# mpc001/auto_avsr

Measured on AMD Instinct MI355X. Metric: video-frames/sec/node (25fps 88x88, max-frames=1600), E2E training step (fwd+bwd+clip+AdamW), higher is better.
Workload: dtype f16 activations x f16x2 weights (atrunk3, atrunk4, decoder, encoder, trunk3, trunk4) + split-bf16 (everything else) forward / bf16 backward

## Files before the change

auto_avsr_amd/csrc/gemm_split.hip:

```cpp
#include "gemm_core.h"
#include "avsr_hip.h"

namespace {

using avsr_gemm_impl::Params;

template <int BM, int BN, int STAGES, int CV, bool BSP = false, int WGM = 2, int WGN = 2, int ACV = 0>
struct SplitKernel {
    static constexpr int BK = 32, NW = WGM * WGN, NTHR = 64 * NW;
    static_assert(NW == 4 || NW == 8, "four or eight waves");
    static constexpr int WM = BM / WGM, WN = BN / WGN, TM = WM / 32, TN = WN / 32;
    static_assert(WM % 32 == 0 && WN % 32 == 0, "wave tile must be a multiple of 32 x 32");
    static constexpr int A_BYTES = BM * 128, B_BYTES = BN * 128, STAGE_BYTES = A_BYTES + B_BYTES;
    static constexpr int A_LOADS = BM / (8 * NW), B_LOADS = BN / (8 * NW);
    static_assert(A_LOADS >= 1 && B_LOADS >= 1 && BM % (8 * NW) == 0 && BN % (8 * NW) == 0, "tile / wave-count mismatch");
    static constexpr int LPT = A_LOADS + B_LOADS;
    static constexpr size_t RING_BYTES = (size_t)STAGES * STAGE_BYTES, EPI_BYTES = (size_t)BM * (BN + 4) * 4;
    static constexpr size_t LDS_BYTES = RING_BYTES > EPI_BYTES ? RING_BYTES : EPI_BYTES;
    static_assert(BM % 64 == 0 && BN % 64 == 0, "tile must be a multiple of 64 x 64");

    struct Rows {
        const float* a[A_LOADS];
        uint32_t mask[A_LOADS];
        const float* b[B_LOADS];
    };

    static AVSR_DEV Rows decode_rows(const Params& p, const float* A, const float* B, int m0, int n0, int wave, int lane) {
        Rows ri;
        const int rsub = lane >> 3, pc = lane & 7;
#pragma unroll
        for (int i = 0; i < A_LOADS; i++) {
            const int r = (wave * A_LOADS + i) * 8 + rsub;
            const int c = pc ^ ((r >> 1) & 7);
            if (CV == 0) {
                const int gr = min(m0 + r, p.M - 1);
                ri.a[i] = A + (size_t)gr * p.lda + c * 4;
                ri.mask[i] = 0;
            } else {
                const int m = min(m0 + r, p.M - 1);
                const int pix = p.cOH * p.cOW;
                const int n = m / pix, rem = m - n * pix;
                const int oh = rem / p.cOW, ow = rem - oh * p.cOW;
                const int ya = oh * p.cS - p.cPH, xa = ow * p.cS - p.cPW;
                ri.a[i] = A + ((long)n * p.cH * p.cW + (long)ya * p.cW + xa) * p.cC + c * 4;
                uint32_t mk = 0;
                for (int t = 0; t < p.cKH * p.cKW; t++) {
                    const int ta = t / p.cKW, tb = t - ta * p.cKW;
                    const int y = ya + ta, x = xa + tb;
                    if (y >= 0 && y < p.cH && x >= 0 && x < p.cW) mk |= 1u << t;
                }
                ri.mask[i] = mk;
            }
        }
#pragma unroll
        for (int i = 0; i < B_LOADS; i++) {
            const int r = (wave * B_LOADS + i) * 8 + rsub;
            const int c = pc ^ ((r >> 1) & 7);
            const int gr = min(n0 + r, p.N - 1);
            ri.b[i] = B + (size_t)gr * p.ldb + c * 4;
        }
        return ri;
    }

    static AVSR_DEV void issue(const Params& p, const Rows& ri, int kbeg, int t, char* stage, int wave) {
        long da, db;
        int tap = 0;
        if (CV == 0) {
            da = db = kbeg + t * BK;
        } else {
            const int cpt = p.cC / BK;
            tap = t / cpt;
            const int cb = (t - tap * cpt) * BK;
            const int ta = tap / p.cKW, tb = tap - ta * p.cKW;
            da = (long)(ta * p.cW + tb) * p.cC + cb;
            db = (long)tap * p.cC + cb;
        }
#pragma unroll
        for (int i = 0; i < A_LOADS; i++) {
            const float* src = ri.a[i] + da;
            if (CV != 0) src = ((ri.mask[i] >> tap) & 1u) ? src : reinterpret_cast<const float*>(p.gate);
            glds16(src, stage + (wave * A_LOADS + i) * 1024);
        }
#pragma unroll
        for (int i = 0; i < B_LOADS; i++) glds16(ri.b[i] + db, stage + A_BYTES + (wave * B_LOADS + i) * 1024);
    }

    static AVSR_DEV Frag<2> frag(const char* base, int r, int half8) {
        const int sw = (r >> 1) & 7;
        const f32x4 a = *reinterpret_cast<const f32x4*>(base + r * 128 + (((2 * half8) ^ sw) << 4));
        const f32x4 b = *reinterpret_cast<const f32x4*>(base + r * 128 + (((2 * half8 + 1) ^ sw) << 4));
        Frag<2> f;
#pragma unroll
        for (int e = 0; e < 4; e++) {
            bf16_t s0[2], s1[2];
            split_bf16<2>(a[e], s0);
            split_bf16<2>(b[e], s1);
            f.p[0][e] = (short)s0[0];
            f.p[1][e] = (short)s0[1];
            f.p[0][e + 4] = (short)s1[0];
            f.p[1][e + 4] = (short)s1[1];
        }
        return f;
    }

    static AVSR_DEV Frag<2> frag_presplit(const char* base, int r, int half8) {
        const int sw = (r >> 1) & 7;
        Frag<2> f;
        f.p[0] = *reinterpret_cast<const bf16x8*>(base + r * 128 + (((2 * half8) ^ sw) << 4));
        f.p[1] = *reinterpret_cast<const bf16x8*>(base + r * 128 + (((2 * half8 + 1) ^ sw) << 4));
        return f;
    }
    static AVSR_DEV void convert_a(char* As) {
#pragma unroll
        for (int j = 0; j < BM * 4 / NTHR; j++) {
            const int idx = threadIdx.x + NTHR * j;
            const int r = idx >> 2, g = idx & 3;
            const Frag<2> f = frag(As, r, g);
            const int sw = (r >> 1) & 7;
            *reinterpret_cast<bf16x8*>(As + r * 128 + (((2 * g) ^ sw) << 4)) = f.p[0];
            *reinterpret_cast<bf16x8*>(As + r * 128 + (((2 * g + 1) ^ sw) << 4)) = f.p[1];
        }
    }

    static AVSR_DEV void run(const Params& p, char* smem) {
        const float* A = reinterpret_cast<const float*>(p.A);
        const float* B = reinterpret_cast<const float*>(p.B);
        const int lane = threadIdx.x & 63, wave = wave_id();
        const int wm = wave / WGN, wn = wave % WGN;
        const int m0 = blockIdx.y * BM, n0 = blockIdx.x * BN;
        const int zs = blockIdx.z;
        int kbeg = 0, nt;
        if (CV == 0) {
            kbeg = zs * p.k_chunk;
            nt = (min(p.K, kbeg + p.k_chunk) - kbeg) / BK;
        } else {
            nt = p.cKH * p.cKW * (p.cC / BK);
        }
        f32x16 acc[TM][TN];
#pragma unroll
        for (int i = 0; i < TM; i++)
#pragma unroll
            for (int j = 0; j < TN; j++)
#pragma unroll
                for (int r = 0; r < 16; r++) acc[i][j][r] = 0.f;

        const Rows ri = decode_rows(p, A, B, m0, n0, wave, lane);
#pragma unroll
        for (int s = 0; s < STAGES - 1; s++)
            if (s < nt) issue(p, ri, kbeg, s, smem + s * STAGE_BYTES, wave);

        auto step = [&](int t, auto issue_flag) {
            constexpr bool ISSUE = decltype(issue_flag)::value;
            if (ISSUE) {
                wait_vmcnt<(STAGES - 2) * LPT>();
            } else {
                switch (nt - 1 - t) {
                    case 0: wait_vmcnt<0>(); break;
                    default: wait_vmcnt<(STAGES > 2 ? LPT : 0)>(); break;
                }
            }
            block_barrier_raw();
            char* As = smem + (t % STAGES) * STAGE_BYTES;
            const char* Bs = As + A_BYTES;
            if (ACV == 1) {
                convert_a(As);
                lds_wait<0>();
                sched_fence();
                block_barrier_raw();
            }
            const int arow = wm * WM + (lane & 31), brow = wn * WN + (lane & 31);
            Frag<2> fa[TM], fb[TN];
            auto load_frags = [&](int ks) {
                const int h8 = ks * 2 + (lane >> 5);
#pragma unroll
                for (int i = 0; i < TM; i++) fa[i] = ACV ? frag_presplit(As, arow + i * 32, h8) : frag(As, arow + i * 32, h8);
#pragma unroll
                for (int j = 0; j < TN; j++) fb[j] = BSP ? frag_presplit(Bs, brow + j * 32, h8) : frag(Bs, brow + j * 32, h8);
            };
            load_frags(0);
            sched_fence();
            if (ISSUE) issue(p, ri, kbeg, t + STAGES - 1, smem + ((t + STAGES - 1) % STAGES) * STAGE_BYTES, wave);
            sched_fence();
#pragma unroll
            for (int ks = 0; ks < BK / 16; ks++) {
#pragma unroll
                for (int i = 0; i < TM; i++)
#pragma unroll
                    for (int j = 0; j < TN; j++) acc[i][j] = mfma32(fa[i].p[1], fb[j].p[0], acc[i][j]);
#pragma unroll
                for (int i = 0; i < TM; i++)
#pragma unroll
                    for (int j = 0; j < TN; j++) acc[i][j] = mfma32(fa[i].p[0], fb[j].p[1], acc[i][j]);
#pragma unroll
                for (int i = 0; i < TM; i++)
#pragma unroll
                    for (int j = 0; j < TN; j++) acc[i][j] = mfma32(fa[i].p[0], fb[j].p[0], acc[i][j]);
                if (ks + 1 < BK / 16) load_frags(ks + 1);
            }
        };
        int t = 0;
        for (; t + STAGES - 1 < nt; t++) step(t, std::true_type{});
        for (; t < nt; t++) step(t, std::false_type{});
        if (CV != 0) {
            Params q = p;
            q.gate = nullptr;
            avsr_gemm_impl::epilogue_lds<BM, BN, TM, TN, NTHR, 1>(acc, q, m0, n0, wm * WM, wn * WN, zs, 0, smem);
            if (BM > 128 && p.colstat && blockIdx.x == 0) {
                const int r2 = (int)gridDim.y + (int)blockIdx.y;
                if (r2 < p.colstat_rows)
                    for (int i = threadIdx.x; i < 2 * p.N; i += NTHR) p.colstat[(size_t)r2 * 2 * p.N + i] = 0.f;
            }
        } else {
            avsr_gemm_impl::epilogue_lds<BM, BN, TM, TN, NTHR, 1>(acc, p, m0, n0, wm * WM, wn * WN, zs, 0, smem);
        }
    }
};

template <int BM, int BN, int STAGES, int CV, bool BSP, int WGM, int WGN, int ACV>
__global__ __launch_bounds__(64 * WGM * WGN) void gemm_split_kernel(Params p) {
    AVSR_DYN_SMEM(smem);
    SplitKernel<BM, BN, STAGES, CV, BSP, WGM, WGN, ACV>::run(p, smem);
}

template <int BM, int BN, int STAGES, int CV, bool BSP, int WGM = 2, int WGN = 2, int ACV = 0>
void launch_split(Params& p, int split_k, hipStream_t stream) {
    using K = SplitKernel<BM, BN, STAGES, CV, BSP, WGM, WGN, ACV>;
    if (CV == 0) {
        int kc = (p.K + split_k - 1) / split_k;
        kc = ((kc + 31) / 32) * 32;
        split_k = (p.K + kc - 1) / kc;
        p.k_chunk = kc;
    } else {
        split_k = 1;
    }
    dim3 grid((p.N + BN - 1) / BN, (p.M + BM - 1) / BM, split_k), block(K::NTHR);
    AVSR_LAUNCH((gemm_split_kernel<BM, BN, STAGES, CV, BSP, WGM, WGN, ACV>), grid, block, K::LDS_BYTES, stream, p);
}

template <int CV, bool BSP>
bool launch_tile(int tile, Params& p, int split_k, hipStream_t stream) {
    switch (tile) {
        case 11: launch_split<64, 64, 3, CV, BSP, 2, 2, 1>(p, split_k, stream); return true;
        case 12: launch_split<64, 64, 2, CV, BSP, 2, 2, 1>(p, split_k, stream); return true;
        case 13: launch_split<128, 64, 2, CV, BSP, 2, 2, 1>(p, split_k, stream); return true;
        case 14: launch_split<128, 128, 2, CV, BSP, 2, 2, 1>(p, split_k, stream); return true;
        case 15: launch_split<128, 64, 3, CV, BSP, 2, 2, 1>(p, split_k, stream); return true;
        case 16: launch_split<128, 128, 3, CV, BSP, 2, 2, 1>(p, split_k, stream); return true;
        case 23: if constexpr (BSP) { launch_split<128, 64, 2, CV, BSP, 2, 2, 2>(p, split_k, stream); return true; } return false;
        case 24: if constexpr (BSP) { launch_split<128, 128, 2, CV, BSP, 2, 2, 2>(p, split_k, stream); return true; } return false;
        case 25: if constexpr (BSP) { launch_split<128, 64, 3, CV, BSP, 2, 2, 2>(p, split_k, stream); return true; } return false;
        case 26: if constexpr (BSP) { launch_split<128, 128, 3, CV, BSP, 2, 2, 2>(p, split_k, stream); return true; } return false;
        case 27: if constexpr (BSP) { launch_split<256, 64, 2, CV, BSP, 4, 2, 2>(p, split_k, stream); return true; } return false;
        case 28: if constexpr (BSP) { launch_split<256, 64, 3, CV, BSP, 4, 2, 2>(p, split_k, stream); return true; } return false;
        case 29: if constexpr (BSP) { launch_split<256, 128, 3, CV, BSP, 4, 2, 2>(p, split_k, stream); return true; } return false;
        case 30: if constexpr (BSP) { launch_split<256, 128, 2, CV, BSP, 4, 2, 2>(p, split_k, stream); return true; } return false;
        case 1: launch_split<64, 64, 3, CV, BSP>(p, split_k, stream); return true;
        case 2: launch_split<64, 64, 2, CV, BSP>(p, split_k, stream); return true;
        case 3: launch_split<128, 64, 2, CV, BSP>(p, split_k, stream); return true;
        case 4: launch_split<128, 128, 2, CV, BSP>(p, split_k, stream); return true;
        case 5: launch_split<128, 64, 3, CV, BSP>(p, split_k, stream); return true;
        case 6: launch_split<128, 128, 3, CV, BSP>(p, split_k, stream); return true;
        case 7: launch_split<128, 64, 2, CV, BSP, 4, 1>(p, split_k, stream); return true;
        default: return false;
    }
}

__global__ __launch_bounds__(256) void split_pack_kernel(const float* __restrict__ src, bf16_t* __restrict__ dst, long n8) {
    for (long i = (long)blockIdx.x * 256 + threadIdx.x; i < n8; i += (long)gridDim.x * 256) {
        float v[8];
        load8(src + i * 8, v);
        bf16x8 hi, lo;
#pragma unroll
        for (int e = 0; e < 8; e++) {
            bf16_t pl[2];
            split_bf16<2>(v[e], pl);
            hi[e] = (short)pl[0];
            lo[e] = (short)pl[1];
        }
        *reinterpret_cast<bf16x8*>(dst + i * 16) = hi;
        *reinterpret_cast<bf16x8*>(dst + i * 16 + 8) = lo;
    }
}
struct AvsrSplitEntry {
    const float* src;
    bf16_t* dst;
    long n8;
    long blk0;
};
__global__ __launch_bounds__(256) void multi_split_pack_kernel(const AvsrSplitEntry* __restrict__ table, int n) {
    int lo_ = 0, hi_ = n - 1;
    while (lo_ < hi_) {
        const int mid = (lo_ + hi_ + 1) >> 1;
        if (table[mid].blk0 <= (long)blockIdx.x) lo_ = mid; else hi_ = mid - 1;
    }
    const AvsrSplitEntry e = table[lo_];
    const long i = ((long)blockIdx.x - e.blk0) * 256 + threadIdx.x;
    if (i >= e.n8) return;
    float v[8];
    load8(e.src + i * 8, v);
    bf16x8 hi, lo;
#pragma unroll
    for (int k = 0; k < 8; k++) {
        bf16_t pl[2];
        split_bf16<2>(v[k], pl);
        hi[k] = (short)pl[0];
        lo[k] = (short)pl[1];
    }
    *reinterpret_cast<bf16x8*>(e.dst + i * 16) = hi;
    *reinterpret_cast<bf16x8*>(e.dst + i * 16 + 8) = lo;
}

}

extern "C" int avsr_gemm_f32s_nt(const float* A, int lda, const float* B, int ldb, int M, int N, int K, const float* bias,
                                 int act, const void* gate, int gate_dtype, int ldg, float gate_scale, float drop_p,
                                 uint64_t seed, const uint64_t* seed_dev, float alpha, const float* alpha_dev,
                                 const void* resid, int resid_dtype, int ldr, void* C, int c_dtype, int ldc, int accumulate,
                                 int split_k, int tile, float* colsum, int b_split, void* c2, int ldc2, hipStream_t stream) {
    AVSR_REQUIRE(!(colsum && accumulate), "gemm_f32s_nt: colsum needs a non-accumulating output");
    AVSR_REQUIRE(!(c2 && (accumulate || c_dtype != 0)), "gemm_f32s_nt: the bf16 twin needs a non-accumulating f32 output");
    AVSR_REQUIRE(K > 0 && K % 64 == 0, "gemm_f32s_nt: K must be a positive multiple of 64");
    AVSR_REQUIRE(lda % 4 == 0 && ldb % 4 == 0, "gemm_f32s_nt: lda/ldb must be multiples of 4 elements");
    AVSR_REQUIRE(((uintptr_t)A % 16) == 0 && ((uintptr_t)B % 16) == 0, "gemm_f32s_nt: operands must be 16-byte aligned");
    AVSR_REQUIRE(!(accumulate && c_dtype != 0), "gemm_f32s_nt: accumulate needs an f32 output");
    AVSR_REQUIRE(!(split_k > 1 && !accumulate), "gemm_f32s_nt: split-K needs accumulate=1");
    if (M <= 0 || N <= 0) return 0;
    Params p{};
    p.A = A; p.B = B; p.lda = lda; p.ldb = ldb;
    p.M = M; p.N = N; p.K = K;
    p.bias = bias; p.act = act;
    p.gate = gate; p.gate_dtype = gate_dtype; p.ldg = ldg; p.gate_scale = gate_scale;
    p.drop_p = drop_p; p.seed = seed; p.seed_dev = seed_dev;
    p.alpha = alpha; p.alpha_dev = alpha_dev;
    p.resid = reinterpret_cast<const float*>(resid); p.resid_dtype = resid_dtype; p.ldr = ldr;
    p.C = C; p.c_dtype = c_dtype; p.ldc = ldc; p.accumulate = accumulate;
    p.colsum = colsum;
    p.C2 = c2; p.ldc2 = ldc2;
    p.nsplit = 1; p.batch_h = 1; p.nbatch = 1;
    if (split_k < 1) split_k = 1;
    float* colsum_det = nullptr;
    if (avsr_det()) {
        split_k = 1;
        if (colsum) {
            AVSR_REQUIRE(ldc == N, "gemm_f32s_nt (deterministic mode): colsum needs a dense output");
            colsum_det = colsum;
            p.colsum = nullptr;
        }
    }
    if (tile == 0) {
        const long t128 = (long)((M + 127) / 128) * ((N + 127) / 128);
        const long t12864 = (long)((M + 127) / 128) * ((N + 63) / 64);
        tile = t128 >= 1024 ? 14 : (t12864 >= 400 ? 13 : 11);
    }
    const bool ok = b_split ? launch_tile<0, true>(tile, p, split_k, stream) : launch_tile<0, false>(tile, p, split_k, stream);
    AVSR_REQUIRE(ok, "gemm_f32s_nt: unknown tile code");
    if (colsum_det) avsr_colsum_det(C, c_dtype, ldc, M, N, colsum_det, stream);
    AVSR_CHECK_LAUNCH("gemm_f32s_nt");
    return 0;
}

static int conv2d_f32s_impl(const float* x, const float* wp, float* y, const void* zero_page, int N, int H, int W, int Cin, int Cout, int KH,
                            int KW, int stride, int pad_h, int pad_w, int tile, int w_split, void* y2, float* stats_part, int stats_tiles,
                            hipStream_t stream) {
    const int OH = (H + 2 * pad_h - KH) / stride + 1, OW = (W + 2 * pad_w - KW) / stride + 1;
    AVSR_REQUIRE(Cin % 64 == 0, "conv2d_f32s: input channel count must be a multiple of 64");
    AVSR_REQUIRE(zero_page != nullptr, "conv2d_f32s: zero page required");
    AVSR_REQUIRE(KH * KW <= 32, "conv2d_f32s: at most 32 filter taps");
    AVSR_REQUIRE((long)N * H * W < (1l << 31) && (long)N * OH * OW < (1l << 31), "conv2d_f32s: pixel count exceeds int32");
    AVSR_REQUIRE(stats_part == nullptr || (long)stats_tiles * 128 >= (long)N * OH * OW, "conv2d_f32s: statistics buffer too small");
    if (N <= 0) return 0;
    Params p{};
    p.A = x; p.B = wp;
    p.K = KH * KW * Cin; p.lda = Cin; p.ldb = p.K;
    p.alpha = 1.f; p.gate_scale = 1.f;
    p.nsplit = 1; p.batch_h = 1; p.nbatch = 1;
    p.gate = zero_page;
    p.c_dtype = 0; p.C = y;
    p.C2 = y2; p.ldc2 = Cout;
    p.cN = N;
    p.cKH = KH; p.cKW = KW; p.cS = stride; p.cPH = pad_h; p.cPW = pad_w; p.cC = Cin;
    p.M = N * OH * OW; p.N = Cout; p.ldc = Cout;
    p.cH = H; p.cW = W; p.cOH = OH; p.cOW = OW;
    p.colstat = stats_part;
    p.colstat_rows = stats_tiles;
    if (tile == 0) tile = Cout >= 128 ? 14 : 13;
    if (tile == 23 && avsr_tune_knobs[21] == 0 && Cout == 64 && (long)N * OH * OW >= 65536) tile = 27;
    if (tile == 23 && avsr_tune_knobs[21] > 0) tile = avsr_tune_knobs[21];
    if (tile == 24 && avsr_tune_knobs[22] > 0) tile = avsr_tune_knobs[22];
    AVSR_REQUIRE(stats_part == nullptr || tile == 13 || tile == 14 || (tile >= 23 && tile <= 30), "conv2d_f32s: statistics need a 128- or 256-row tile");
    const bool ok = w_split ? launch_tile<1, true>(tile, p, 1, stream) : launch_tile<1, false>(tile, p, 1, stream);
    AVSR_REQUIRE(ok, "conv2d_f32s: unknown tile code");
    AVSR_CHECK_LAUNCH("conv2d_f32s");
    return 0;
}

extern "C" int avsr_conv2d_f32s(const float* x, const float* wp, float* y, const void* zero_page, int N, int H, int W, int Cin,
                                int Cout, int KH, int KW, int stride, int pad_h, int pad_w, int tile, int w_split, void* y2,
                                hipStream_t stream) {
    return conv2d_f32s_impl(x, wp, y, zero_page, N, H, W, Cin, Cout, KH, KW, stride, pad_h, pad_w, tile, w_split, y2, nullptr, 0, stream);
}

extern "C" int avsr_conv2d_f32s_stats(const float* x, const float* wp, float* y, const void* zero_page, int N, int H, int W, int Cin,
                                      int Cout, int KH, int KW, int stride, int pad_h, int pad_w, int tile, int w_split, void* y2,
                                      float* stats_part, int stats_tiles, hipStream_t stream) {
    AVSR_REQUIRE(stats_part != nullptr, "conv2d_f32s_stats: statistics buffer required");
    return conv2d_f32s_impl(x, wp, y, zero_page, N, H, W, Cin, Cout, KH, KW, stride, pad_h, pad_w, tile, w_split, y2, stats_part, stats_tiles, stream);
}

extern "C" int avsr_split_pack(const float* src, void* dst, int64_t n, hipStream_t stream) {
    AVSR_REQUIRE(n % 8 == 0, "split_pack: element count must be a multiple of 8");
    AVSR_REQUIRE(((uintptr_t)src % 16) == 0 && ((uintptr_t)dst % 16) == 0, "split_pack: 16-byte aligned buffers");
    if (n <= 0) return 0;
    const long n8 = n / 8, nb = (n8 + 255) / 256;
    AVSR_LAUNCH(split_pack_kernel, dim3((unsigned)(nb > 4096 ? 4096 : nb)), dim3(256), 0, stream, src, (bf16_t*)dst, n8);
    AVSR_CHECK_LAUNCH("split_pack");
    return 0;
}

extern "C" int avsr_multi_split_pack(const void* table, int n, int total_blocks, hipStream_t stream) {
    if (n <= 0 || total_blocks <= 0) return 0;
    AVSR_LAUNCH(multi_split_pack_kernel, dim3(total_blocks), dim3(256), 0, stream, reinterpret_cast<const AvsrSplitEntry*>(table), n);
    AVSR_CHECK_LAUNCH("multi_split_pack");
    return 0;
}
```

Baseline: 69900.

## Add persistent direct 3x3 C64 split-bf16 conv kernel with halo patch staging

Adds a dedicated persistent kernel for 3x3 stride-1 64-to-64 channel convolutions with split-bf16 weights. It keeps the high weight half in registers and the low half in LDS, and stages haloed input row-bands into a double-buffered, swizzled LDS patch. The patch loads are woven into the MFMA loop, and the epilogue fuses the bf16 copy and BN statistics. It replaces the generic implicit-GEMM tile path, cutting redundant im2col loads and weight reloads. The cost is a complex hand-scheduled kernel with heavy register use and large LDS.

```diff
diff --git a/auto_avsr_amd/csrc/conv3x3_c64_split.hip b/auto_avsr_amd/csrc/conv3x3_c64_split.hip
--- /dev/null
+++ b/auto_avsr_amd/csrc/conv3x3_c64_split.hip
@@ -0,0 +1,330 @@
+#include "prims.h"
+#include "avsr_hip.h"
+
+namespace {
+
+template <class T> AVSR_DEV void opaque(T& v) {
+#ifndef AVSR_EMU
+    asm volatile("" : "+v"(v));
+#endif
+}
+AVSR_DEV void wave_lds_sync() {
+#ifdef AVSR_EMU
+    (void)__shfl_xor(0, 1);
+#else
+    __builtin_amdgcn_fence(__ATOMIC_SEQ_CST, "wavefront");
+    __builtin_amdgcn_wave_barrier();
+#endif
+}
+
+constexpr int C = 64, KSTEPS = 9 * C / 16, HSTEPS = KSTEPS / 2;
+constexpr int PIX_BYTES = C * 4;
+constexpr int WROW_BYTES = 9 * C * 4;
+constexpr int NTHR = 256, NWAVE = 4;
+constexpr int WLO_BYTES = KSTEPS * C * 32;
+constexpr int STRIP_BYTES = 16 * 128;
+constexpr int MEET_BYTES = NWAVE * 2 * 32 * 4;
+constexpr int LDS_LIMIT = 160 * 1024;
+constexpr int PR_LIMIT = (LDS_LIMIT - WLO_BYTES - NWAVE * STRIP_BYTES - MEET_BYTES) / 2 / 1024 * 8;
+constexpr int DMA_PER_WAVE = (PR_LIMIT / 8 + NWAVE - 1) / NWAVE;
+
+struct C64SParams {
+    const char* src;
+    const char* wq;
+    float* y;
+    bf16_t* y2;
+    float* stats;
+    const void* zero;
+    int N, H, W, R, bands, ntiles;
+    int patch_bytes;
+    int stats_rows, group, ngroups;
+};
+
+__global__ __launch_bounds__(NTHR) void conv3x3_split_c64_kernel(C64SParams p) {
+    AVSR_DYN_SMEM(smem);
+    char* wlo = smem + 2 * p.patch_bytes;
+    const int lane = threadIdx.x & 63, wave = wave_id();
+    char* strip = wlo + WLO_BYTES + wave * STRIP_BYTES;
+    float* meet = reinterpret_cast<float*>(wlo + WLO_BYTES + NWAVE * STRIP_BYTES);
+    const int mg = wave >> 1, ng = wave & 1;
+    const int W2 = p.W + 2, prows = (p.R + 2) * W2;
+    const int khalf = lane >> 5;
+    const int G = (int)gridDim.x;
+
+    bf16x8 wh[KSTEPS];
+    {
+        const char* wrow = p.wq + (size_t)(ng * 32 + (lane & 31)) * WROW_BYTES + 32 * khalf;
+#pragma unroll
+        for (int s = 0; s < KSTEPS; s++) wh[s] = *reinterpret_cast<const bf16x8*>(wrow + 64 * s);
+    }
+    for (int idx = threadIdx.x; idx < KSTEPS * C * 2; idx += NTHR) {
+        const int s = idx >> 7, kh = (idx >> 6) & 1, n = idx & 63;
+        *reinterpret_cast<bf16x8*>(wlo + idx * 16) = *reinterpret_cast<const bf16x8*>(p.wq + (size_t)n * WROW_BYTES + 64 * s + 32 * kh + 16);
+    }
+#pragma unroll
+    for (int s = 0; s < KSTEPS; s++) opaque(wh[s]);
+    __syncthreads();
+    int wlo_ofs = khalf * 1024 + (ng * 32 + (lane & 31)) * 16;
+
+    const int step_y = (8 * NWAVE) / W2, step_x = 8 * NWAVE - step_y * W2;
+    int py0, px0;
+    {
+        const int pr = wave * 8 + (lane >> 3);
+        py0 = pr / W2;
+        px0 = pr - py0 * W2;
+    }
+    struct Stager {
+        const char* base;
+        char* buf;
+        int y0, py, px;
+    };
+    auto stage_begin = [&](int tile, int half, char* buf) {
+        const int n = tile / p.bands, y0 = (tile - n * p.bands) * p.R;
+        return Stager{p.src + ((size_t)n * p.H + y0) * p.W * PIX_BYTES + half * 128, buf, y0, py0, px0};
+    };
+    auto stage_one = [&](Stager& st, int i) {
+        const int j = wave + NWAVE * i;
+        if (j * 8 >= prows) return;
+        const int pr = j * 8 + (lane >> 3);
+        const int c = (lane & 7) ^ ((pr >> 1) & 7);
+        const int yy = st.y0 - 1 + st.py;
+        const bool ok = pr < prows && st.px >= 1 && st.px <= p.W && yy >= 0 && yy < p.H;
+        const void* src = ok ? (const void*)(st.base + ((st.py - 1) * p.W + (st.px - 1)) * PIX_BYTES + c * 16) : p.zero;
+        glds16(src, st.buf + j * 1024);
+        st.px += step_x;
+        st.py += step_y;
+        if (st.px >= W2) {
+            st.px -= W2;
+            st.py++;
+        }
+    };
+
+    int fbase[9][4];
+#pragma unroll
+    for (int i = 0; i < 4; i++) {
+        int pix = mg * 128 + 32 * i + (lane & 31);
+        if (pix >= p.R * p.W) pix = 0;
+        const int y = pix / p.W, x = pix - y * p.W;
+#pragma unroll
+        for (int tap = 0; tap < 9; tap++) {
+            const int pr = y * W2 + x + (tap / 3) * W2 + (tap % 3);
+            fbase[tap][i] = (pr * 128) ^ (((pr >> 1) & 7) << 4) ^ (khalf << 5);
+        }
+    }
+
+    struct Band {
+        size_t g0;
+        int npix;
+    };
+    auto band_of = [&](int tile) {
+        const int n = tile / p.bands, y0 = (tile - n * p.bands) * p.R;
+        return Band{((size_t)n * p.H + y0) * p.W, min(p.R, p.H - y0) * p.W};
+    };
+    float cs[4], cq[4];
+#pragma unroll
+    for (int e = 0; e < 4; e++) cs[e] = cq[e] = 0.f;
+    auto stats_meet = [&]() {
+#pragma unroll
+        for (int m = 32; m >= 8; m >>= 1)
+#pragma unroll
+            for (int e = 0; e < 4; e++) {
+                cs[e] += __shfl_xor(cs[e], m);
+                cq[e] += __shfl_xor(cq[e], m);
+            }
+        if (lane < 8)
+#pragma unroll
+            for (int e = 0; e < 4; e++) {
+                meet[(wave * 2 + 0) * 32 + lane * 4 + e] = cs[e];
+                meet[(wave * 2 + 1) * 32 + lane * 4 + e] = cq[e];
+            }
+#pragma unroll
+        for (int e = 0; e < 4; e++) cs[e] = cq[e] = 0.f;
+        lds_wait<0>();
+        sched_fence();
+    };
+    auto stats_row = [&](int row) {
+        if (threadIdx.x < 2 * C) {
+            const int j = threadIdx.x >> 6, c = threadIdx.x & 63, w0 = c >> 5, cc = c & 31;
+            p.stats[(size_t)row * 2 * C + threadIdx.x] = meet[(w0 * 2 + j) * 32 + cc] + meet[((w0 + 2) * 2 + j) * 32 + cc];
+        }
+    };
+
+    int tile = blockIdx.x;
+    if (tile < p.ntiles) {
+        Stager st = stage_begin(tile, 0, smem);
+#pragma unroll
+        for (int i = 0; i < DMA_PER_WAVE; i++) stage_one(st, i);
+        wait_vmcnt<0>();
+    }
+    int it = 0, pending_row = -1;
+    static_assert(DMA_PER_WAVE <= HSTEPS, "the woven pieces must fit the k-steps");
+    for (; tile < p.ntiles; tile += G, it++) {
+        const bool more = tile + G < p.ntiles;
+        f32x16 acc[4];
+#pragma unroll
+        for (int i = 0; i < 4; i++)
+#pragma unroll
+            for (int r = 0; r < 16; r++) acc[i][r] = 0.f;
+#pragma unroll
+        for (int h = 0; h < 2; h++) {
+            const char* patch = smem + h * p.patch_bytes;
+#pragma unroll
+            for (int tap = 0; tap < 9; tap++)
+#pragma unroll
+                for (int i = 0; i < 4; i++) opaque(fbase[tap][i]);
+            opaque(wlo_ofs);
+            if (h == 1) wait_vmcnt<0>();
+            block_barrier_raw();
+            if (h == 0 && pending_row >= 0) {
+                stats_row(pending_row);
+                pending_row = -1;
+            }
+            const bool do_stage = h == 0 || more;
+            Stager st = stage_begin(h == 0 || !more ? tile : tile + G, 1 - h, smem + (1 - h) * p.patch_bytes);
+
+            i32x4 xh[2][4], xl[2][4], wl[2];
+            auto req_x = [&](int t, int i, int plane) {
+                return lds_read16_async(patch + (fbase[t >> 1][i] ^ ((t & 1) << 6) ^ (plane << 4)));
+            };
+            auto req_w = [&](int t) { return lds_read16_async(wlo + wlo_ofs + 2048 * (4 * (t >> 1) + 2 * h + (t & 1))); };
+#pragma unroll
+            for (int t = 0; t < 2; t++) {
+#pragma unroll
+                for (int i = 0; i < 4; i++) xl[t][i] = req_x(t, i, 1);
+                wl[t] = req_w(t);
+#pragma unroll
+                for (int i = 0; i < 4; i++) xh[t][i] = req_x(t, i, 0);
+            }
+#pragma unroll
+            for (int t = 0; t < HSTEPS; t++) {
+                if (t + 1 < HSTEPS) lds_wait<9>();
+                else lds_wait<0>();
+                const int s = 4 * (t >> 1) + 2 * h + (t & 1), cur = t & 1;
+                const bool ahead = t + 2 < HSTEPS;
+#pragma unroll
+                for (int i = 0; i < 4; i++) {
+                    lds_tie(xh[cur][i]);
+                    lds_tie(xl[cur][i]);
+                }
+                lds_tie(wl[cur]);
+#pragma unroll
+                for (int i = 0; i < 4; i++) {
+                    acc[i] = mfma32(wh[s], __builtin_bit_cast(bf16x8, xl[cur][i]), acc[i]);
+                    sched_fence();
+                    if (ahead) xl[cur][i] = req_x(t + 2, i, 1);
+                    sched_fence();
+                }
+                const bf16x8 wlc = __builtin_bit_cast(bf16x8, wl[cur]);
+#pragma unroll
+                for (int i = 0; i < 4; i++) {
+                    acc[i] = mfma32(wlc, __builtin_bit_cast(bf16x8, xh[cur][i]), acc[i]);
+                    sched_fence();
+                    if (i == 3 && ahead) wl[cur] = req_w(t + 2);
+                    if (i == 1 && t < DMA_PER_WAVE && do_stage) stage_one(st, t);
+                    sched_fence();
+                }
+#pragma unroll
+                for (int i = 0; i < 4; i++) {
+                    acc[i] = mfma32(wh[s], __builtin_bit_cast(bf16x8, xh[cur][i]), acc[i]);
+                    sched_fence();
+                    if (ahead) xh[cur][i] = req_x(t + 2, i, 0);
+                    sched_fence();
+                }
+            }
+        }
+        wait_vmcnt<0>();
+        const Band b = band_of(tile);
+#pragma unroll
+        for (int i = 0; i < 4; i++)
+#pragma unroll
+            for (int hf = 0; hf < 2; hf++) {
+                if (((lane >> 4) & 1) == hf) {
+                    const int r = lane & 15;
+#pragma unroll
+                    for (int q = 0; q < 4; q++)
+                        *reinterpret_cast<f32x4*>(strip + r * 128 + (((2 * q + khalf) ^ ((r >> 1) & 7)) << 4)) =
+                            f32x4{acc[i][4 * q], acc[i][4 * q + 1], acc[i][4 * q + 2], acc[i][4 * q + 3]};
+                }
+                wave_lds_sync();
+                f32x4 vv[2];
+#pragma unroll
+                for (int rr = 0; rr < 2; rr++) {
+                    const int r = (lane >> 3) + 8 * rr, ch = lane & 7;
+                    vv[rr] = *reinterpret_cast<const f32x4*>(strip + r * 128 + ((ch ^ ((r >> 1) & 7)) << 4));
+                }
+#pragma unroll
+                for (int rr = 0; rr < 2; rr++) {
+                    const int r = (lane >> 3) + 8 * rr, ch = lane & 7;
+                    const f32x4 v = vv[rr];
+                    const int pix = mg * 128 + 32 * i + 16 * hf + r;
+                    if (pix < b.npix) {
+                        const size_t o = (b.g0 + pix) * C + ng * 32 + ch * 4;
+                        *reinterpret_cast<f32x4*>(p.y + o) = v;
+                        if (p.y2)
+                            *reinterpret_cast<bf16x4*>(p.y2 + o) = bf16x4{(short)f2bf(v[0]), (short)f2bf(v[1]), (short)f2bf(v[2]), (short)f2bf(v[3])};
+                        if (p.stats) {
+#pragma unroll
+                            for (int e = 0; e < 4; e++) {
+                                cs[e] += v[e];
+                                cq[e] += v[e] * v[e];
+                            }
+                        }
+                    }
+                }
+                wave_lds_sync();
+            }
+        if (p.stats && (!more || it % p.group == p.group - 1)) {
+            stats_meet();
+            pending_row = (int)blockIdx.x + G * (it / p.group);
+        }
+    }
+    if (p.stats) {
+        block_barrier_raw();
+        if (pending_row >= 0) stats_row(pending_row);
+        if (threadIdx.x < 2 * C) {
+            for (int g = it > 0 ? (it - 1) / p.group + 1 : 0; g < p.ngroups; g++)
+                p.stats[((size_t)blockIdx.x + (size_t)G * g) * 2 * C + threadIdx.x] = 0.f;
+            for (int r = G * p.ngroups + (int)blockIdx.x; r < p.stats_rows; r += G) p.stats[(size_t)r * 2 * C + threadIdx.x] = 0.f;
+        }
+    }
+}
+
+int patch_bytes_of(int H, int W, int* R_out) {
+    int R = 256 / W;
+    if (R > H) R = H;
+    while (R > 0 && (R + 2) * (W + 2) > PR_LIMIT) R--;
+    if (R_out) *R_out = R;
+    return ((R + 2) * (W + 2) * 128 + 1023) / 1024 * 1024;
+}
+
+}
+
+int avsr_conv3x3_c64_split_supported(int H, int W) {
+    if (W < 4 || W > 254 || H < 1) return 0;
+    int R;
+    patch_bytes_of(H, W, &R);
+    return R >= 1;
+}
+
+int avsr_conv3x3_c64_split_launch(const void* x, const void* wq, float* y, void* y2, float* stats_part, int stats_rows,
+                                  const void* zero_page, int N, int H, int W, hipStream_t stream) {
+    C64SParams p{};
+    p.src = (const char*)x; p.wq = (const char*)wq; p.y = y; p.y2 = (bf16_t*)y2;
+    p.stats = stats_rows > 0 ? stats_part : nullptr;
+    p.zero = zero_page;
+    p.N = N; p.H = H; p.W = W;
+    p.patch_bytes = patch_bytes_of(H, W, &p.R);
+    p.bands = (H + p.R - 1) / p.R;
+    p.ntiles = N * p.bands;
+    int grid = p.ntiles < 256 ? p.ntiles : 256;
+    p.stats_rows = stats_rows; p.group = 1; p.ngroups = 0;
+    if (p.stats) {
+        if (grid > stats_rows) grid = stats_rows;
+        const int iters = (p.ntiles + grid - 1) / grid, max_groups = stats_rows / grid;
+        p.group = (iters + max_groups - 1) / max_groups;
+        p.ngroups = (iters + p.group - 1) / p.group;
+    }
+    const size_t lds = 2 * (size_t)p.patch_bytes + WLO_BYTES + NWAVE * STRIP_BYTES + MEET_BYTES;
+    AVSR_LAUNCH(conv3x3_split_c64_kernel, dim3(grid), dim3(NTHR), lds, stream, p);
+    return 0;
+}
diff --git a/auto_avsr_amd/csrc/gemm_split.hip b/auto_avsr_amd/csrc/gemm_split.hip
--- a/auto_avsr_amd/csrc/gemm_split.hip
+++ b/auto_avsr_amd/csrc/gemm_split.hip
@@ -359,6 +359,10 @@
     return 0;
 }
 
+int avsr_conv3x3_c64_split_supported(int H, int W);
+int avsr_conv3x3_c64_split_launch(const void* x, const void* wq, float* y, void* y2, float* stats_part, int stats_rows,
+                                  const void* zero_page, int N, int H, int W, hipStream_t stream);
+
 static int conv2d_f32s_impl(const float* x, const float* wp, float* y, const void* zero_page, int N, int H, int W, int Cin, int Cout, int KH,
                             int KW, int stride, int pad_h, int pad_w, int tile, int w_split, void* y2, float* stats_part, int stats_tiles,
                             hipStream_t stream) {
@@ -384,6 +388,13 @@
     p.colstat = stats_part;
     p.colstat_rows = stats_tiles;
     if (tile == 0) tile = Cout >= 128 ? 14 : 13;
+    if (tile == 23 && avsr_tune_knobs[21] == 0 && avsr_tune_knobs[27] != 1 && w_split && KH == 3 && KW == 3 && stride == 1 && pad_h == 1 &&
+        pad_w == 1 && Cin == 64 && Cout == 64 && ((long)N * OH * OW >= 65536 || avsr_tune_knobs[27] == 2) &&
+        avsr_conv3x3_c64_split_supported(H, W)) {
+        avsr_conv3x3_c64_split_launch(x, wp, y, y2, stats_part, stats_part ? stats_tiles : 0, zero_page, N, H, W, stream);
+        AVSR_CHECK_LAUNCH("conv2d_f32s");
+        return 0;
+    }
     if (tile == 23 && avsr_tune_knobs[21] == 0 && Cout == 64 && (long)N * OH * OW >= 65536) tile = 27;
     if (tile == 23 && avsr_tune_knobs[21] > 0) tile = avsr_tune_knobs[21];
     if (tile == 24 && avsr_tune_knobs[22] > 0) tile = avsr_tune_knobs[22];
```

After: 70670, median of 6. 1.1% higher.
